# francescofugazzi/3dgsconverter

Measured on AMD Instinct MI355X. Metric: Msplats/sec SOR k=16, higher is better.
Workload: dtype f32 select / f64 finalize

## Files before the change

3dgsconverter_amd/_lib.py:

```python
from __future__ import annotations

import contextlib
import ctypes as C
import functools
import os
import re
import threading
import time

import numpy as np

_HERE = os.path.dirname(os.path.abspath(__file__))
LIB_PATH = os.environ.get("GSX_LIB_PATH") or os.path.join(_HERE, "libgsx_hip.so")

KNN_AUTO, KNN_BRUTE, KNN_GRID, KNN_TREE = 0, 1, 2, 3
PROBE_ROOT_DIST2, PROBE_ROOT_DSQRT = 0, 1
PROBE_MEAN_NET, PROBE_MEAN_LIST, PROBE_MEAN_LE128, PROBE_MEAN_NP = 0, 1, 2, 3
T_SOR_KNN, T_SOR_BIN, T_SOR_FALLBACK, T_SOR_STATS, T_DENSITY, T_KMEANS_ASSIGN, T_KMEANS_UPDATE, T_QUANTIZE = range(8)
T_SLAB_PREP, T_SLAB_ROWS, T_SLAB_MEANS, T_SLAB_COLL = range(8, 12)


class GsxError(RuntimeError):
    """Raised for every failure of the HIP path (missing library, no GPU, HIP error)."""

# ... 223 lines not shown
    "gsx_dev_download_staged": (_I, [_P, _P, _P, C.c_size_t]),
    "gsx_host_gather_f32": (_I, [_P, _I64, _I64, C.POINTER(_I64), _I, _P]),
    "gsx_host_gather_columns_f32": (_I, [_P, _I64, _I64, C.POINTER(_I64), _I, _P]),
    "gsx_host_compact_rows": (_I, [_P, _I64, _I64, _P, _P, _I64, C.POINTER(_I64)]),
    "gsx_host_take_rows": (_I, [_P, _I64, _I64, _P, _I64, _P]),
    "gsx_host_zero_columns": (_I, [_P, _I64, _I64, C.POINTER(_I64), _I]),
    "gsx_host_append_columns": (_I, [_P, _I64, _I64, _P, _I64, _P, _I64]),
    "gsx_host_take_rows_append": (_I, [_P, _I64, _I64, _P, _I64, _P, _I64, _P, _I64]),
    "gsx_host_take_rows_shape": (_I, [_P, _I64, _I64, _P, _I64, _P, _I64, C.POINTER(_I64), _I, _P, _I64]),
    "gsx_rgb_from_sh": (_I, [_P, _I64, _P, _P]),
    "gsx_rgb_from_sh_dev": (_I, [_P, _P, _I64, _P, _P]),
    "gsx_rgb_from_sh_list": (_I, [_P, _I64, _P, _P, _I64, C.POINTER(_I64)]),
    "gsx_rgb_from_sh_list_dev": (_I, [_P, _P, _I64, _P, _P, _I64, _P]),
    "gsx_compact_rows_dev": (_I, [_P, _P, _P, _P, _I64, _P, _P, C.POINTER(_I64)]),
    "gsx_mask_bbox_dev": (_I, [_P, _P, _I64, _P, _P]),
    "gsx_mask_ge_dev": (_I, [_P, _P, _P, _I64, _D, _P]),
    "gsx_sor_knn_dev": (_I, [_P, _P, _P, _P, _I64, _I64, _I64, _I64, _I, _I, _P, C.POINTER(SorInfo)]),
    "gsx_sor_knn_share_dev": (_I, [_P, _P, _P, _P, _I64, _I64, _I, _I, _I, _I, _P, C.POINTER(SorInfo)]),
    "gsx_sor_debug_brick_plan": (_I, [_P, _P, _P, _P, _I64]),
    "gsx_sor_debug_work_queue": (_I, [_P, _P, _P, _P]),
    "gsx_sor_debug_tree": (_I, [_P, _P, _P, _P, _I64, C.POINTER(_I64), C.POINTER(_I64)]),
    "gsx_sor_debug_wave_stamps": (_I, [_P, _I, _P, _I64, _P]),
    "gsx_sor_debug_points_per_cell": (_D, [_I, _I64, _I]),
    "gsx_sor_debug_group_bricks": (_I, [_P, _I64, _I, _I, _I, _P, C.POINTER(C.c_int32)]),
    "gsx_sor_debug_refine_sizing": (_I, [C.POINTER(RefineSizingIn), C.POINTER(RefineSizingOut)]),
    "gsx_knn_probe_root_dev": (_I, [_P, _P, _I64, _I, _P]),
    "gsx_knn_probe_mean_dev": (_I, [_P, _P, _I64, _I64, _I, _I, _I, _P]),
    "gsx_sor_stats_dev": (_I, [_P, _P, _I64, _D, _P]),
    "gsx_sor_mask_dev": (_I, [_P, _P, _I64, _P, _P]),
    "gsx_comm_unique_id": (_I, [_P]),
    "gsx_comm_init": (_I, [_P, _I, _I, _P]),
    "gsx_comm_destroy": (_I, [_P]),
    "gsx_comm_all_reduce": (_I, [_P, _P, _I64, _I]),
    "gsx_comm_all_gather": (_I, [_P, _P, _P, _I64]),
    "gsx_comm_all_to_all_v": (_I, [_P, _P, _P, _P, _P, _P, _P, _I]),
    "gsx_comm_all_to_all_segs": (_I, [_P, _P, _P, _I, _P, _P, _P, _P, _I]),
    "gsx_comm_abort": (_I, [_P]),
    "gsx_comm_transport": (_I, [_P]),
    "gsx_comm_rank": (_I, [_P, C.POINTER(_I), C.POINTER(_I)]),
    "gsx_comm_barrier": (_I, [_P]),
    "gsx_slab_plan": (_I, [_P, _I, _I, _I64, _I, _D, C.POINTER(SlabPlan)]),
    "gsx_sor_slab_step_dev": (_I, [_P, _P, _I64, _I, _D, _D, _P, C.POINTER(SlabStep)]),
    "gsx_slab_bbox_dev": (_I, [_P, _P, _P, _P, _I64, _I64, _P]),
    "gsx_slab_hist_dev": (_I, [_P, _P, _P, _P, _I64, _I64, _P, _P]),
    "gsx_slab_partition_dev": (_I, [_P, _P, _P, _P, _I64, _I64, _I, _I, C.c_float, C.c_float, _P, _I, _P, _P, _P, _P, _P]),
    "gsx_sor_knn_slab_dev": (_I, [_P, _P, _I64, _I64, _I, _P, _P]),
# ... 1985 lines not shown
        if sh_count:
            sh = np.stack([data["f_rest_%d" % j][rows] for j in range(sh_count)], axis=1)
            if level == 2:
                out["sh"] = np.clip((sh - -2.0) / (2.0 - -2.0) * 255, 0, 255).astype(np.uint8)
            else:
                out["sh"] = sh.astype(out.dtype["sh"].base)
    return out


def ksplat_centres_host(data: np.ndarray, bucket_size: int) -> np.ndarray:
    idx = np.arange(0, len(data), bucket_size)
    cols = []
    with np.errstate(all="ignore"):
        for a in "xyz":
            v = data[a]
            cols.append((np.minimum.reduceat(v, idx) + np.maximum.reduceat(v, idx)) / 2.0)
    return np.column_stack(cols).astype(np.float32)


def grid_points_per_cell(k: int, n: int, tuned: bool) -> float:
    return float(load().gsx_sor_debug_points_per_cell(int(k), int(n), int(bool(tuned))))


def grid_group_bricks(bricks, nbx: int, nby: int, nbz: int):
    b = np.array(bricks, dtype=np.uint32)
    sizes = np.zeros(8, np.uint32)
    ng = C.c_int32()
    check(load().gsx_sor_debug_group_bricks(b.ctypes.data, b.size, int(nbx), int(nby), int(nbz), sizes.ctypes.data, C.byref(ng)),
          "gsx_sor_debug_group_bricks")
    return b, [int(v) for v in sizes[:ng.value]]


def grid_refine_sizing(qb_lo, qb_hi, sub_queries: int, n_sub: int, pts_per_cell: float, parent_h: float, adaptive: int, hist,
                       bin_vol: float) -> RefineSizingOut:
    a = RefineSizingIn((C.c_float * 3)(*qb_lo), (C.c_float * 3)(*qb_hi), int(sub_queries), int(n_sub), float(pts_per_cell),
                       float(parent_h), int(adaptive), (C.c_uint32 * 32)(*[int(v) for v in hist]), float(bin_vol))
    out = RefineSizingOut()
    check(load().gsx_sor_debug_refine_sizing(C.byref(a), C.byref(out)), "gsx_sor_debug_refine_sizing")
    return out


def np_exp_host(x: np.ndarray) -> np.ndarray:
    x = np.ascontiguousarray(x, dtype=np.float32)
    out = np.empty_like(x)
    check(load().gsx_np_expf_host(x.ctypes.data, out.ctypes.data, x.size), "gsx_np_expf_host")
    return out
# ... 1659 lines not shown
```

3dgsconverter_amd/csrc/api.hip:

```cpp
#include <algorithm>
#include <mutex>

#include "grid_policy.h"
#include "gsx_common.h"
#include "gsx_internal.h"
#include "sor_grid_params.h"

namespace gsx {

static thread_local std::string g_err;

void set_error(const char *fmt, ...)
{
    char buf[1024];
    va_list ap;
    va_start(ap, fmt);
    vsnprintf(buf, sizeof(buf), fmt, ap);
    va_end(ap);
    g_err = buf;
}

int DevBuf::reserve(size_t bytes)
{
    if (bytes <= cap) return 0;
// ... 191 lines not shown
        s.used = 0;
        s.launches = 0;
        s.total_ms = 0.0;
    }
    return 0;
}

int gsx_ctx_get_timing(gsx_ctx *c, int slot, uint64_t *launches, double *total_ms)
{
    if (!c || slot < 0 || slot >= GSX_T_SLOTS) GSX_FAIL("gsx_ctx_get_timing: bad arguments");
    GSX_HIP(hipStreamSynchronize(c->stream));
    GSX_CHECK(timing_resolve(c, slot));
    if (launches) *launches = c->slots[slot].launches;
    if (total_ms) *total_ms = c->slots[slot].total_ms;
    return 0;
}

int gsx_ctx_set_param(gsx_ctx *c, const char *name, double value)
{
    if (!c || !name) GSX_FAIL("gsx_ctx_set_param: bad arguments");
    if (!strcmp(name, "grid_points_per_cell")) {
        if (value != 0.0 && !(value >= 1.0 && value <= 512.0)) GSX_FAIL("grid_points_per_cell must be 0 (auto) or in [1,512]");
        c->grid_points_per_cell = value;
    } else if (!strcmp(name, "brute_below")) {
        c->brute_below = (int64_t)value;
    } else if (!strcmp(name, "debug_skip")) {
#ifdef GSX_ABLATE
        c->debug_skip = (int)value;
#else
        if (value != 0.0) GSX_FAIL("debug_skip needs a profiling build of the library (-DGSX_ABLATE); this one computes exact results only");
#endif
    } else if (!strcmp(name, "kmeans_mfma")) {
        c->kmeans_mfma = value != 0.0;
    } else if (!strcmp(name, "km_exact_blocks")) {
        c->km_exact_blocks = value < 1 ? 1 : (value > 32 ? 32 : (int)value);
    } else if (!strcmp(name, "km_seg_rows")) {
        c->km_seg_rows = value >= 64 ? 64 : (value >= 32 ? 32 : 16);
    } else if (!strcmp(name, "km_group_mb")) {
        c->km_group_mb = value < 0 ? 0 : (int)value;
    } else if (!strcmp(name, "kmeans_cs")) {
        c->kmeans_cs = value != 0.0;
    } else if (!strcmp(name, "km_small_wgs")) {
        c->km_small_wgs = (int)value;
    } else if (!strcmp(name, "kmeans_cs_small")) {
        c->kmeans_cs_small = value != 0.0;
    } else if (!strcmp(name, "ring_fast")) {
// ... 157 lines not shown
#ifdef GSX_WAVE_STAMPS
    gsx::KnnWs &w = c->ws[0];
    if (!w.wavestamps.p) GSX_FAIL("gsx_sor_debug_wave_stamps: no grid KNN call has run on this context");
    GSX_HIP(hipSetDevice(c->device));
    GSX_HIP(hipStreamSynchronize(c->stream));
    const int64_t slots = c->ws_cap;
    const int64_t m = std::min<int64_t>(slots, cap);
    if (m > 0)
        GSX_HIP(hipMemcpy(out, (const uint64_t *)w.wavestamps.p + (size_t)kernel * slots * gsx::WS_WORDS,
                          sizeof(uint64_t) * gsx::WS_WORDS * (size_t)m, hipMemcpyDeviceToHost));
    *count = slots;
    return 0;
#else
    (void)cap;
    GSX_FAIL("gsx_sor_debug_wave_stamps needs a diagnostic build of the library (-DGSX_WAVE_STAMPS)");
#endif
}

double gsx_sor_debug_points_per_cell(int k, int64_t n, int tuned)
{
    return tuned ? gsx::grid_pts_per_cell(k, n) : gsx::grid_pts_per_cell_base(k, n);
}

int gsx_sor_debug_group_bricks(uint32_t *bricks, int64_t count, int nbx, int nby, int nbz, uint32_t *group_sizes, int32_t *n_groups)
{
    if (!bricks || !group_sizes || !n_groups || count < 0 || count > UINT32_MAX || nbx < 1 || nby < 1 || nbz < 1)
        GSX_FAIL("gsx_sor_debug_group_bricks: bad arguments");
    for (int64_t i = 0; i < count; ++i)
        if ((uint64_t)bricks[i] >= (uint64_t)nbx * nby * nbz) GSX_FAIL("gsx_sor_debug_group_bricks: brick %u outside the grid", bricks[i]);
    const std::vector<unsigned> sizes = gsx::group_deferred_bricks(bricks, (unsigned)count, nbx, nby, nbz);
    for (int g = 0; g < gsx::GRID_MAX_GROUPS; ++g) group_sizes[g] = g < (int)sizes.size() ? sizes[g] : 0u;
    *n_groups = (int32_t)sizes.size();
    return 0;
}

int gsx_sor_debug_refine_sizing(const gsx_refine_sizing_in *in, gsx_refine_sizing_out *out)
{
    if (!in || !out) GSX_FAIL("gsx_sor_debug_refine_sizing: null argument");
    const gsx::RefineClip r = gsx::refine_clip(in->qb_lo, in->qb_hi, in->sub_queries, in->pts_per_cell, in->parent_h, in->adaptive);
    *out = gsx_refine_sizing_out{r.nd3, r.probe_g, r.h_est, r.M, r.cert, {r.lo[0], r.lo[1], r.lo[2]}, {r.hi[0], r.hi[1], r.hi[2]}, r.r_cert,
                                 r.probe_g ? gsx::refine_probe_edge(in->hist, in->bin_vol, in->qb_lo, in->qb_hi, r.r_cert, in->n_sub,
                                                                    r.h_est, in->pts_per_cell)
                                           : 0.0};
    return 0;
}

// ... 504 lines not shown
```

3dgsconverter_amd/csrc/grid_policy.h:

```cpp
#pragma once

#include <algorithm>
#include <cmath>
#include <cstdint>
#include <unordered_map>
#include <vector>

namespace gsx {

constexpr int MAX_BUCKETS = 4096;
constexpr int MAX_BUCKET_CELLS = 4096;
constexpr int64_t GRID_MAX_CELLS = (int64_t)MAX_BUCKETS * MAX_BUCKET_CELLS - 64;

inline double grid_fill(int64_t n) { return n >= 4000000 ? 54.0 : 58.0; }

inline double grid_pts_per_cell_base(int k, int64_t n)
{
    double m = std::max(2.0, 0.47 * (double)(k + 1));
    const double fill = grid_fill(n);
    for (int cells = 8; cells >= 1; cells /= 2)
        if (m * cells > fill && m * cells <= 66.0) m = fill / cells;
    return m;
}

inline double grid_pts_per_cell(int k, int64_t n)
{
    double m = grid_pts_per_cell_base(k, n);
    const double fill = grid_fill(n);
    if (k >= 17 && k <= 20) m = std::min(m, fill / 8.0 + 0.375 * (double)std::max(0, k - 18));
    if (k >= 26 && k <= 31) m = std::min(m, 12.0 * fill / 54.0);
    if (k >= 35 && k <= 43) m = std::min(m, (k <= 38 ? 13.5 : 14.5) * fill / 54.0);
    if (k >= 44 && k <= 62) m = std::min(m, k <= 49 ? 16.0 : (k <= 58 ? 22.0 : 24.0));
    return m;
}

inline int64_t grid_cell_cap(int64_t n_ref) { return std::max<int64_t>(n_ref / 2, 64) + 64; }
inline int64_t grid_refine_cell_cap(int64_t n_ref) { return std::min<int64_t>(std::max<int64_t>(4 * n_ref, 64), GRID_MAX_CELLS) + 64; }

struct HistVerdict {
    unsigned fullest = 0, nonzero = 0;
    bool to_tree = false;
    bool no_deferral = false;
};
inline HistVerdict grid_hist_verdict(const unsigned *starts , int64_t n_ref, int nshares)
{
    HistVerdict v;
    for (int b = 0; b < MAX_BUCKETS; ++b) {
        const unsigned c = starts[b + 1] >= starts[b] ? starts[b + 1] - starts[b] : 0u;
        v.fullest = std::max(v.fullest, c);
        v.nonzero += c > 0;
    }
    v.to_tree = v.nonzero > 0 && (double)v.fullest > 3.0 * (double)n_ref / (double)v.nonzero;
    v.no_deferral = v.nonzero > 0 && (double)v.fullest <= 1.5 * (double)n_ref / (double)v.nonzero && nshares == 1;
    return v;
}

struct PlanCall {
    bool enabled;
    int level;
    bool whole_cloud;
// ... 120 lines not shown
```

3dgsconverter_amd/csrc/gsx_common.h:

```cpp
#pragma once

#include <hip/hip_runtime.h>

#include <cstdarg>
#include <cstdint>
#include <cstdio>
#include <cstring>
#include <string>
#include <vector>

#include "../../include/gsx_hip.h"
#include "dev_carve.h"

namespace gsx {

constexpr int WAVE = 64;

void set_error(const char *fmt, ...);

#define GSX_HIP(call)                                                                         \
    do {                                                                                      \
        hipError_t e__ = (call);                                                              \
        if (e__ != hipSuccess) {                                                              \
            gsx::set_error("%s failed: %s (%s:%d)", #call, hipGetErrorString(e__), __FILE__,  \
// ... 105 lines not shown
    PinnedBuf host;
};

struct TimingSlot {
    std::vector<hipEvent_t> ev;
    size_t used = 0;
    uint64_t launches = 0;
    double total_ms = 0.0;
};

}

struct gsx_ctx {
    int device = 0;
    hipStream_t stream = nullptr;
    hipStream_t owned_stream = nullptr;
    bool timing = false;
    unsigned timing_mask = 0xffffffffu;
    gsx::TimingSlot slots[GSX_T_SLOTS];
    int num_cu = 256;
    void *comm = nullptr;

    double grid_points_per_cell = 0.0;
    int64_t brute_below = 2048;
    int debug_skip = 0;
    int adaptive = 0;
    int defer_words = 64;
    int last_knn_algo = 0;
    int tree = 1;
    int kmeans_mfma = 1;
    int tree_leaf_cap = 0;
    int tree_cand_limit = 0;
    double tree_near_cell = 0.5;
    int tree_last_leaf_cap = 0;
    double tree_scale = 0.0;
    int km_exact_blocks = 4;
    int km_seg_rows = 32;
    int km_group_mb = 0;
    int km_small_wgs = 0;
    int kmeans_cs_small = 1;
    int kmeans_cs = 1;
    int ring_fast = 1;
    int phase2_net = 1;
    int brick_plan = 1;
    int ws_cap = 0;
    int wq_grid[4] = {0, 0, 0, 0};
// ... 30 lines not shown
```

3dgsconverter_amd/csrc/sor_grid.hip:

```cpp
#include <algorithm>
#include <chrono>
#include <cmath>
#include <cstdlib>
#include <type_traits>
#include <unordered_map>
#include <vector>

#include "grid_policy.h"
#include "gsx_common.h"
#include "gsx_internal.h"
#include "knn_common.h"
#include "knn_mfma.h"
#include "sor_grid_params.h"

namespace gsx {


constexpr int MAX_DIM = 1024;
#ifndef GSX_BUCKET_POINTS
#define GSX_BUCKET_POINTS 4096
#endif
constexpr int BUCKET_POINTS = GSX_BUCKET_POINTS;
#ifndef GSX_BIN_TILE
#define GSX_BIN_TILE 8192
#endif
constexpr int BIN_TILE = GSX_BIN_TILE;
constexpr int BRICK_THREADS = 256;
constexpr int HEAVY_RING_CANDIDATES = 1 << 16;
constexpr int HEAVY_CHUNK = 32768;
#ifndef GSX_WCAP_BIG
#define GSX_WCAP_BIG 32
#endif
#ifndef GSX_WCAP_MID
#define GSX_WCAP_MID 24
#endif
constexpr int WCAP = 24;

struct GridParamArgs {
    int n;
    double pts_per_cell;
    int cell_cap, debug_skip, share, nshares, defer_words;
    float parent_h;
    GridParams *gp;
    unsigned *devflags;
    double h_hint;
    int cert_axis;
    float cert_lo, cert_hi;
    unsigned *cert_count;
    int plan_req = 0, plan_cap = 0;
#ifdef GSX_WAVE_STAMPS
    unsigned long long *stamps = nullptr;
    int stamps_cap = 0;
#endif
};
__device__ void grid_params_body(const float *part, int nparts, const GridParamArgs &a);

__global__ __launch_bounds__(256) void bbox_partial_kernel(const float *__restrict__ x, const float *__restrict__ y,
                                                           const float *__restrict__ z, int64_t stride, int n,
                                                           float *__restrict__ part, GridParamArgs gpa)
{
    __shared__ float red[7][4];
    float mn[3] = {__builtin_inff(), __builtin_inff(), __builtin_inff()};
    float mx[3] = {-__builtin_inff(), -__builtin_inff(), -__builtin_inff()};
    float bad = 0.0f;
    const int step = gridDim.x * blockDim.x;
    for (int64_t i0 = blockIdx.x * blockDim.x + threadIdx.x; i0 < n; i0 += 4 * (int64_t)step) {
        float v[4][3];
#pragma unroll
        for (int u = 0; u < 4; ++u) {
            const int64_t i = (int64_t)(i0 + u * step < n ? i0 + u * step : i0) * stride;
            v[u][0] = x[i];
            v[u][1] = y[i];
            v[u][2] = z[i];
        }
#pragma unroll
        for (int u = 0; u < 4; ++u)
#pragma unroll
            for (int a = 0; a < 3; ++a) {
                mn[a] = fminf(mn[a], v[u][a]);
                mx[a] = fmaxf(mx[a], v[u][a]);
                bad = (fabsf(v[u][a]) < __builtin_inff()) ? bad : 1.0f;
            }
    }
#pragma unroll
    for (int a = 0; a < 3; ++a)
#pragma unroll
        for (int off = 32; off > 0; off >>= 1) {
            mn[a] = fminf(mn[a], __shfl_xor(mn[a], off));
            mx[a] = fmaxf(mx[a], __shfl_xor(mx[a], off));
// ... 65 lines not shown
        emax = e[a] > emax ? e[a] : emax;
    }
    double h;
    if (nd == 0 || !(emax < 1e300)) {
        h = 1.0;
    } else {
        double per = vol * pts_per_cell / (double)(n > 0 ? n : 1);
        h = nd == 3 ? cbrt(per) : (nd == 2 ? sqrt(per) : per);
        if (a.h_hint > 0.0 && a.h_hint < h) h = a.h_hint;
        double hmin = emax / (double)(MAX_DIM - 1);
        if (!(h > hmin)) h = hmin;
    }
    int nx, ny, nz;
    int bg = 1, bny = 1, bnz = 1;
    long long padded = 0;
    float inv_h;
    for (int it = 0; it < 256; ++it) {
        inv_h = (float)(1.0 / h);
        nx = (int)((v[3] - v[0]) * inv_h) + 1;
        ny = (int)((v[4] - v[1]) * inv_h) + 1;
        nz = (int)((v[5] - v[2]) * inv_h) + 1;
        bool ok = nx <= MAX_DIM && ny <= MAX_DIM && nz <= MAX_DIM && nx > 0 && ny > 0 && nz > 0;
        if (ok) {
            double per_row = (double)nx * pts_per_cell;
            bg = (int)(sqrt((double)BUCKET_POINTS / (per_row > 1.0 ? per_row : 1.0)) + 0.5);
            if (bg < 1) bg = 1;
            if (bg > (ny > nz ? ny : nz)) bg = ny > nz ? ny : nz;
            while (bg > 1 && (long long)bg * bg * nx > MAX_BUCKET_CELLS) --bg;
            for (;;) {
                bny = (ny + bg - 1) / bg;
                bnz = (nz + bg - 1) / bg;
                if ((long long)bny * bnz <= MAX_BUCKETS) break;
                ++bg;
            }
            padded = (long long)bny * bnz * bg * bg * nx;
            ok = (long long)bg * bg * nx <= MAX_BUCKET_CELLS && padded <= (long long)cell_cap;
        }
        if (ok) break;
        h *= 1.1;
    }
    bool bad = v[6] > 0.0f;
    for (int a = 0; a < 6; ++a) bad |= !(fabsf(v[a]) < 3.0e38f);
    if (bad || !(nx > 0 && ny > 0 && nz > 0) || padded <= 0 || padded > (long long)cell_cap ||
        (long long)bg * bg * nx > MAX_BUCKET_CELLS) {
        bad = true;
        nx = ny = nz = 1;
        bg = bny = bnz = 1;
        inv_h = 0.0f;
    }
    gp->ox = v[0]; gp->oy = v[1]; gp->oz = v[2];
    gp->inv_h = inv_h;
    gp->h = (float)h;
    gp->nx = nx; gp->ny = ny; gp->nz = nz;
    gp->bk_g = bg; gp->bk_ny = bny; gp->bk_nz = bnz;
    gp->bk_count = bny * bnz;
    gp->bk_cells = bg * bg * nx;
    gp->ncells = gp->bk_count * gp->bk_cells;
    int bdx = 2, bdy = 2, bdz = 2;
    if (pts_per_cell * 8.0 > 66.0) bdz = 1;
// ... 370 lines not shown
        if (j < hi - lo) {
            const float4 r = stage[j];
            out[tab[bucket_of(g, cell_coord(r.y, g.oy, g.inv_h, g.ny), cell_coord(r.z, g.oz, g.inv_h, g.nz))] + j] = r;
        }
    }
}

#ifndef GSX_SORT_THREADS
#define GSX_SORT_THREADS 512
#endif
#ifndef GSX_SORT_PPT
#define GSX_SORT_PPT 16
#endif
constexpr int SORT_THREADS = GSX_SORT_THREADS;
constexpr int SORT_PPT = GSX_SORT_PPT;
constexpr unsigned SORT_CAP = SORT_THREADS * SORT_PPT;

__device__ __forceinline__ int quarter_coord(float v, float o, float inv_h, int dim)
{
    int c = (int)((v - o) * (4.0f * inv_h));
    return min(max(c, 0), 4 * dim - 1);
}

template <bool FINE>
__global__ __launch_bounds__(SORT_THREADS) void bucket_sort_kernel(const GridParams *__restrict__ gp,
                                                          const unsigned *__restrict__ bk_start,
                                                          const float4 *__restrict__ in, float4 *__restrict__ out,
                                                          unsigned *__restrict__ cell_start, unsigned big_limit,
                                                          unsigned *__restrict__ fine_start)
{
    constexpr int SUB = FINE ? 4 : 1;
    __shared__ unsigned cnt[SUB * MAX_BUCKET_CELLS];
    __shared__ unsigned wsum[SORT_THREADS / 64];
    const GridParams g = *gp;
    const int b = blockIdx.x;
    if (g.bad_input || b >= g.bk_count) return;
    const int ncell = g.bk_cells;
    const int cells = SUB * ncell;
    const unsigned s0 = bk_start[b], s1 = bk_start[b + 1];
    if (b == g.bk_count - 1 && threadIdx.x == 0) {
        cell_start[(size_t)g.bk_count * ncell] = s1;
        if (FINE) fine_start[(size_t)g.bk_count * cells] = s1;
    }
    if (s1 - s0 > big_limit) return;
    const int by = b % g.bk_ny, bz = b / g.bk_ny;
    for (int i = threadIdx.x; i < cells; i += SORT_THREADS) cnt[i] = 0;
    __syncthreads();
    auto local_cell = [&](const float4 p) {
        const int cx = FINE ? quarter_coord(p.x, g.ox, g.inv_h, g.nx) : cell_coord(p.x, g.ox, g.inv_h, g.nx);
        const int cy = cell_coord(p.y, g.oy, g.inv_h, g.ny);
        const int cz = cell_coord(p.z, g.oz, g.inv_h, g.nz);
        return ((cz - bz * g.bk_g) * g.bk_g + (cy - by * g.bk_g)) * (SUB * g.nx) + cx;
    };
    const bool fits = s1 - s0 <= SORT_CAP;
    float4 p[SORT_PPT];
    int cell[SORT_PPT];
    unsigned rk[SORT_PPT];
    if (fits) {
#pragma unroll
        for (int u = 0; u < SORT_PPT; ++u) p[u] = in[min(s0 + u * SORT_THREADS + threadIdx.x, s1 - 1)];
#pragma unroll
        for (int u = 0; u < SORT_PPT; ++u) {
            cell[u] = local_cell(p[u]);
            rk[u] = s0 + u * SORT_THREADS + threadIdx.x < s1 ? atomicAdd(&cnt[cell[u]], 1u) : 0u;
        }
    } else {
        for (unsigned i = s0 + threadIdx.x; i < s1; i += SORT_THREADS) atomicAdd(&cnt[local_cell(in[i])], 1u);
    }
    __syncthreads();
    const int seg = (cells + SORT_THREADS - 1) / SORT_THREADS;
    const int c0 = min(cells, (int)threadIdx.x * seg), c1 = min(cells, c0 + seg);
    unsigned sum = 0;
    for (int c = c0; c < c1; ++c) sum += cnt[c];
    unsigned inc = sum;
#pragma unroll
    for (int off = 1; off < 64; off <<= 1) {
        unsigned o = __shfl_up(inc, off);
        if ((int)(threadIdx.x & 63) >= off) inc += o;
    }
    const int wv = threadIdx.x >> 6;
    if ((threadIdx.x & 63) == 63) wsum[wv] = inc;
    __syncthreads();
    unsigned run = inc - sum;
    for (int i = 0; i < wv; ++i) run += wsum[i];
    __syncthreads();
    for (int c = c0; c < c1; ++c) {
        const unsigned v = cnt[c];
        cnt[c] = run;
        run += v;
    }
    __syncthreads();
    unsigned *cs = cell_start + (size_t)b * ncell;
    for (int i = threadIdx.x; i < ncell; i += SORT_THREADS) cs[i] = s0 + cnt[SUB * i];
    if (FINE) {
        unsigned *fs = fine_start + (size_t)b * cells;
        for (int i = threadIdx.x; i < cells; i += SORT_THREADS) fs[i] = s0 + cnt[i];
    }
    if (fits) {
#pragma unroll
        for (int u = 0; u < SORT_PPT; ++u)
            if (s0 + u * SORT_THREADS + threadIdx.x < s1) out[s0 + cnt[cell[u]] + rk[u]] = p[u];
    } else {
        __syncthreads();
        for (unsigned i = s0 + threadIdx.x; i < s1; i += SORT_THREADS) {
            const float4 q = in[i];
            out[s0 + atomicAdd(&cnt[local_cell(q)], 1u)] = q;
        }
    }
}

constexpr unsigned BIG_BUCKET = 32768;
constexpr int BIG_CHUNK = 8192;

__device__ __forceinline__ int bucket_containing(const unsigned *bk_start, int nb, unsigned pos)
{
    int lo = 0, hi = nb;
    while (hi - lo > 1) {
        const int mid = (lo + hi) >> 1;
        if (bk_start[mid] <= pos) lo = mid; else hi = mid;
    }
    return lo;
}

template <bool SCATTER>
__global__ __launch_bounds__(256) void big_bucket_kernel(const GridParams *__restrict__ gp, const unsigned *__restrict__ bk_start,
                                                         int n, const float4 *__restrict__ in, float4 *__restrict__ out,
                                                         unsigned *cell_start ,
                                                         unsigned *cursor )
{
    __shared__ unsigned cnt[MAX_BUCKET_CELLS];
    __shared__ unsigned base[SCATTER ? MAX_BUCKET_CELLS : 1];
// ... 1907 lines not shown
    if (L.adaptive) {
        GSX_CHECK(w.deferred.reserve(sizeof(unsigned) * (size_t)(cap + 64)));
        GSX_CHECK(w.heavylist.reserve(sizeof(unsigned) * (size_t)std::max<int64_t>(q_count, 1)));
    }
    if (!L.all) {
        GSX_CHECK(w.qsorted.reserve(sizeof(float4) * (size_t)q_count));
        GSX_CHECK(w.qcellstart.reserve(sizeof(unsigned) * (size_t)(cap + 1)));
    }
    L.gp = w.gridparams.as<GridParams>();
    L.refs = w.packed.as<float4>();
    L.rstart = w.cellstart.as<unsigned>();
    L.mfma_ok = ctx->filter_mfma != 0 && n_ref < (int64_t(1) << 28);
    L.plan = grid_plan_eligible({ctx->brick_plan != 0, L.level, L.all, L.slab, L.sk != nullptr, L.nshares, L.k, L.mfma_ok,
                                 ctx->phase2_net != 0, L.pts_per_cell, L.h_hint, L.kth_out != nullptr});
    L.plan_cap = n_ref / 16 + 4096;
    if (L.plan) {
        GSX_CHECK(w.finestart.reserve(sizeof(unsigned) * (size_t)(4 * cap + 4)));
        GSX_CHECK(w.bricklist.reserve(sizeof(uint2) * (size_t)L.plan_cap));
        GSX_CHECK(w.bundleoff.reserve(sizeof(unsigned) * 2 * (size_t)(MAX_DIM / 2) * (MAX_DIM / 2)));
    }
    return 0;
}

static int level_grid_params(GridLevel &L)
{
    gsx_ctx *ctx = L.ctx;
    KnnWs &w = L.w;
    const SlabKnn *sk = L.sk;
    GSX_CHECK(timing_begin(ctx, GSX_T_SOR_BIN));
    GridParamArgs gpa{(int)L.n_ref, L.pts_per_cell, (int)L.cap, ctx->debug_skip, L.share, L.nshares, L.adaptive ? ctx->defer_words : 0,
                      L.parent_h, L.gp, ctx->devflags.as<unsigned>(), L.h_hint, sk ? sk->cert_axis : -1, sk ? sk->cert_lo : 0.0f,
                      sk ? sk->cert_hi : 0.0f, sk ? sk->cert_count : nullptr, L.plan ? 1 : 0, (int)L.plan_cap};
#ifdef GSX_WAVE_STAMPS
    if (L.level == 0) {
        const int ws_cap = ctx->num_cu * 8 * (BRICK_THREADS / 64);
        const size_t ws_bytes = sizeof(unsigned long long) * 2 * (size_t)ws_cap * WS_WORDS;
        GSX_CHECK(w.wavestamps.reserve(ws_bytes));
        GSX_HIP(hipMemsetAsync(w.wavestamps.p, 0, ws_bytes, ctx->stream));
        gpa.stamps = w.wavestamps.as<unsigned long long>();
        gpa.stamps_cap = ws_cap;
        ctx->ws_cap = ws_cap;
    }
#endif
    L.adaptive_at_bbox = L.adaptive;
    if (sk && sk->box.b7)
        hipLaunchKernelGGL(grid_params_known_box_kernel, dim3(1), dim3(64), 0, ctx->stream, sk->box, w.bboxpart.as<float>(), gpa);
    else
        hipLaunchKernelGGL(bbox_partial_kernel, dim3(L.bbox_blocks), dim3(256), 0, ctx->stream, L.x, L.y, L.z, L.stride, (int)L.n_ref,
                           w.bboxpart.as<float>(), gpa);
    GSX_HIP(hipGetLastError());
    if (L.adaptive) GSX_CHECK(w.qcellstart.reserve(sizeof(unsigned) * (size_t)(L.cap + 1)));
    return 0;
}

static int level_histogram(GridLevel &L, bool *done)
{
    gsx_ctx *ctx = L.ctx;
    KnnWs &w = L.w;
    L.tree_ok = (L.adaptive || (L.slab && ctx->adaptive)) && ctx->tree && L.level == 0 && L.k + 1 <= 65 && L.n_ref > L.k;
    if (!L.tree_ok) return 0;
    GSX_CHECK(bin_hist(ctx, w, L.x, L.y, L.z, L.stride, 0, L.n_ref, L.gp));
    static thread_local std::vector<unsigned> starts(MAX_BUCKETS + 1);
    GSX_HIP(hipMemcpyAsync(starts.data(), w.bk_start, sizeof(unsigned) * (MAX_BUCKETS + 1), hipMemcpyDeviceToHost, ctx->stream));
    GSX_HIP(hipStreamSynchronize(ctx->stream));
    const HistVerdict v = grid_hist_verdict(starts.data(), L.n_ref, L.nshares);
    L.hist_done = true;
    if (v.to_tree) {
        GSX_CHECK(timing_end(ctx, GSX_T_SOR_BIN));
        if (L.trace)
            fprintf(stderr, "[gsx] level 0: fullest bucket %u of %lld points in %u buckets -> tree path\n", v.fullest, (long long)L.n_ref, v.nonzero);
        const int rc = launch_knn_tree(ctx, L.x, L.y, L.z, L.stride, L.n_ref, L.q_begin, L.q_count, L.k, L.mean_out, L.kth_out, L.info,
                                       L.slab ? L.ref_only_from : INT32_MAX, L.share, L.nshares, true);
// ... 284 lines not shown
```

include/gsx_hip.h:

```cpp
#ifndef GSX_HIP_H
#define GSX_HIP_H

#include <stddef.h>
#include <stdint.h>

#ifdef __cplusplus
extern "C" {
#endif

typedef struct gsx_ctx gsx_ctx;

enum {
    GSX_KNN_AUTO = 0,
    GSX_KNN_BRUTE = 1,
    GSX_KNN_GRID = 2,
    GSX_KNN_TREE = 3
};

enum {
    GSX_T_SOR_KNN = 0,
    GSX_T_SOR_BIN = 1,
    GSX_T_SOR_FALLBACK = 2,
    GSX_T_SOR_STATS = 3,
    GSX_T_DENSITY = 4,
// ... 69 lines not shown
                            void *out, int64_t out_row_bytes);
int gsx_host_take_rows_append(const void *rows, int64_t row_bytes, int64_t n, const uint32_t *idx, int64_t n_idx,
                              const uint8_t *extra, int64_t extra_bytes, void *out, int64_t out_row_bytes);
int gsx_host_take_rows_shape(const void *rows, int64_t row_bytes, int64_t n, const uint32_t *idx, int64_t n_idx,
                             const uint8_t *extra, int64_t extra_bytes, const int64_t *zero_offsets, int nzero, void *out,
                             int64_t out_row_bytes);

int gsx_mask_bbox_dev(gsx_ctx *ctx, const float *rows_dev, int64_t n, const double *bounds6, uint8_t *mask_dev);
int gsx_mask_ge_dev(gsx_ctx *ctx, const float *vals_dev, const uint32_t *orig_dev, int64_t n, double threshold,
                    uint8_t *mask_dev);

int gsx_sor_knn_dev(gsx_ctx *ctx, const float *x, const float *y, const float *z, int64_t stride,
                    int64_t n_ref, int64_t q_begin, int64_t q_count, int k, int algo,
                    float *mean_out_dev, gsx_sor_info *info );
int gsx_sor_knn_share_dev(gsx_ctx *ctx, const float *x, const float *y, const float *z, int64_t stride,
                          int64_t n, int k, int algo, int share, int nshares, float *mean_out_dev,
                          gsx_sor_info *info );
int gsx_sor_debug_brick_plan(gsx_ctx *ctx, int32_t *grid, float *origin, uint32_t *list, int64_t cap);
int gsx_sor_debug_work_queue(gsx_ctx *ctx, uint32_t *ctr, int64_t *items, int32_t *blocks);
int gsx_sor_debug_tree(gsx_ctx *ctx, uint32_t *counters, uint64_t *keys, uint32_t *leafstart, int64_t cap, int64_t *n_out,
                       int64_t *leaves_out);
int gsx_sor_debug_wave_stamps(gsx_ctx *ctx, int kernel, uint64_t *out, int64_t cap, int64_t *count);
double gsx_sor_debug_points_per_cell(int k, int64_t n, int tuned);
int gsx_sor_debug_group_bricks(uint32_t *bricks, int64_t count, int nbx, int nby, int nbz, uint32_t *group_sizes, int32_t *n_groups);
typedef struct gsx_refine_sizing_in {
    float    qb_lo[3], qb_hi[3];
    uint32_t sub_queries, n_sub;
    double   pts_per_cell;
    float    parent_h;
    int32_t  adaptive;
    uint32_t hist[32];
    double   bin_vol;
} gsx_refine_sizing_in;
typedef struct gsx_refine_sizing_out {
    int32_t nd3, probe_g;
    double  h_est, margin, cert;
    float   clip_lo[3], clip_hi[3], r_cert;
    double  h_hint;
} gsx_refine_sizing_out;
int gsx_sor_debug_refine_sizing(const gsx_refine_sizing_in *in, gsx_refine_sizing_out *out);
enum { GSX_PROBE_ROOT_DIST2 = 0, GSX_PROBE_ROOT_DSQRT = 1 };
int gsx_knn_probe_root_dev(gsx_ctx *ctx, const double *in_dev, int64_t n, int mode, double *out_dev);
enum { GSX_PROBE_MEAN_NET = 0, GSX_PROBE_MEAN_LIST = 1, GSX_PROBE_MEAN_LE128 = 2, GSX_PROBE_MEAN_NP = 3 };
int gsx_knn_probe_mean_dev(gsx_ctx *ctx, const double *d2_dev, int64_t m, int64_t stride, int k, int form, int cap,
                           float *out_dev);
int gsx_sor_stats_dev(gsx_ctx *ctx, const float *mean_dists_dev, int64_t n, double threshold_factor,
// ... 496 lines not shown
```

Before: 6229.

## Vectorize bbox reduction for packed rows and specialize bucket sort per fill

When x, y and z are interleaved with stride 3 and 16-byte aligned, the bbox partial kernel now reads them as float4 rows with unrolled wave-wide loads and un-rotates the per-lane axes afterwards. The bucket sort kernel now dispatches to template instantiations sized to the actual number of points per thread, so under-filled buckets skip wasted register loads. Bucket edge sizing is factored into a shared host/device helper with a runtime bucket_points parameter and a debug entry point. The specialization adds several kernel instantiations, which grows code size and may raise register pressure.

```diff
diff --git a/3dgsconverter_amd/_lib.py b/3dgsconverter_amd/_lib.py
--- a/3dgsconverter_amd/_lib.py
+++ b/3dgsconverter_amd/_lib.py
@@ -269,6 +269,7 @@
     "gsx_sor_debug_tree": (_I, [_P, _P, _P, _P, _I64, C.POINTER(_I64), C.POINTER(_I64)]),
     "gsx_sor_debug_wave_stamps": (_I, [_P, _I, _P, _I64, _P]),
     "gsx_sor_debug_points_per_cell": (_D, [_I, _I64, _I]),
+    "gsx_sor_debug_bucket_edge": (_I, [_I, _I, _I, _D, _I, _I64, _P]),
     "gsx_sor_debug_group_bricks": (_I, [_P, _I64, _I, _I, _I, _P, C.POINTER(C.c_int32)]),
     "gsx_sor_debug_refine_sizing": (_I, [C.POINTER(RefineSizingIn), C.POINTER(RefineSizingOut)]),
     "gsx_knn_probe_root_dev": (_I, [_P, _P, _I64, _I, _P]),
@@ -2300,6 +2301,13 @@
     return float(load().gsx_sor_debug_points_per_cell(int(k), int(n), int(bool(tuned))))
 
 
+def grid_bucket_edge(nx: int, ny: int, nz: int, pts_per_cell: float, bucket_points: int = 0, cell_cap: int = 1 << 40):
+    out = np.zeros(5, np.int64)
+    check(load().gsx_sor_debug_bucket_edge(int(nx), int(ny), int(nz), float(pts_per_cell), int(bucket_points), int(cell_cap),
+                                           out.ctypes.data), "gsx_sor_debug_bucket_edge")
+    return int(out[0]), int(out[1]), int(out[2]), int(out[3]), bool(out[4])
+
+
 def grid_group_bricks(bricks, nbx: int, nby: int, nbz: int):
     b = np.array(bricks, dtype=np.uint32)
     sizes = np.zeros(8, np.uint32)
diff --git a/3dgsconverter_amd/csrc/api.hip b/3dgsconverter_amd/csrc/api.hip
--- a/3dgsconverter_amd/csrc/api.hip
+++ b/3dgsconverter_amd/csrc/api.hip
@@ -237,6 +237,9 @@
     if (!strcmp(name, "grid_points_per_cell")) {
         if (value != 0.0 && !(value >= 1.0 && value <= 512.0)) GSX_FAIL("grid_points_per_cell must be 0 (auto) or in [1,512]");
         c->grid_points_per_cell = value;
+    } else if (!strcmp(name, "bucket_points")) {
+        if (value != 0.0 && !(value >= 64.0 && value <= 1048576.0)) GSX_FAIL("bucket_points must be 0 (built in) or in [64,1048576]");
+        c->bucket_points = (int)value;
     } else if (!strcmp(name, "brute_below")) {
         c->brute_below = (int64_t)value;
     } else if (!strcmp(name, "debug_skip")) {
@@ -440,6 +443,14 @@
     return tuned ? gsx::grid_pts_per_cell(k, n) : gsx::grid_pts_per_cell_base(k, n);
 }
 
+int gsx_sor_debug_bucket_edge(int nx, int ny, int nz, double pts_per_cell, int bucket_points, int64_t cell_cap, int64_t out[5])
+{
+    if (!out || nx < 1 || ny < 1 || nz < 1 || bucket_points < 0) GSX_FAIL("gsx_sor_debug_bucket_edge: bad arguments");
+    const gsx::BucketEdge e = gsx::grid_bucket_edge(nx, ny, nz, pts_per_cell, bucket_points, (long long)cell_cap);
+    out[0] = e.bg; out[1] = e.bny; out[2] = e.bnz; out[3] = e.padded; out[4] = e.ok ? 1 : 0;
+    return 0;
+}
+
 int gsx_sor_debug_group_bricks(uint32_t *bricks, int64_t count, int nbx, int nby, int nbz, uint32_t *group_sizes, int32_t *n_groups)
 {
     if (!bricks || !group_sizes || !n_groups || count < 0 || count > UINT32_MAX || nbx < 1 || nby < 1 || nbz < 1)
diff --git a/3dgsconverter_amd/csrc/grid_policy.h b/3dgsconverter_amd/csrc/grid_policy.h
--- a/3dgsconverter_amd/csrc/grid_policy.h
+++ b/3dgsconverter_amd/csrc/grid_policy.h
@@ -5,6 +5,12 @@
 #include <cstdint>
 #include <unordered_map>
 #include <vector>
+
+#if defined(__HIPCC__)
+#define GSX_POLICY_HD __host__ __device__
+#else
+#define GSX_POLICY_HD
+#endif
 
 namespace gsx {
 
@@ -36,6 +42,34 @@
 
 inline int64_t grid_cell_cap(int64_t n_ref) { return std::max<int64_t>(n_ref / 2, 64) + 64; }
 inline int64_t grid_refine_cell_cap(int64_t n_ref) { return std::min<int64_t>(std::max<int64_t>(4 * n_ref, 64), GRID_MAX_CELLS) + 64; }
+
+#ifndef GSX_BUCKET_POINTS
+#define GSX_BUCKET_POINTS 4096
+#endif
+constexpr int BUCKET_POINTS = GSX_BUCKET_POINTS;
+struct BucketEdge {
+    int bg, bny, bnz;
+    long long padded;
+    bool ok;
+};
+GSX_POLICY_HD inline BucketEdge grid_bucket_edge(int nx, int ny, int nz, double pts_per_cell, int bucket_points, long long cell_cap)
+{
+    BucketEdge e;
+    const double per_row = (double)nx * pts_per_cell;
+    e.bg = (int)(sqrt((double)(bucket_points > 0 ? bucket_points : BUCKET_POINTS) / (per_row > 1.0 ? per_row : 1.0)) + 0.5);
+    if (e.bg < 1) e.bg = 1;
+    if (e.bg > (ny > nz ? ny : nz)) e.bg = ny > nz ? ny : nz;
+    while (e.bg > 1 && (long long)e.bg * e.bg * nx > MAX_BUCKET_CELLS) --e.bg;
+    for (;;) {
+        e.bny = (ny + e.bg - 1) / e.bg;
+        e.bnz = (nz + e.bg - 1) / e.bg;
+        if ((long long)e.bny * e.bnz <= MAX_BUCKETS) break;
+        ++e.bg;
+    }
+    e.padded = (long long)e.bny * e.bnz * e.bg * e.bg * nx;
+    e.ok = (long long)e.bg * e.bg * nx <= MAX_BUCKET_CELLS && e.padded <= cell_cap;
+    return e;
+}
 
 struct HistVerdict {
     unsigned fullest = 0, nonzero = 0;
diff --git a/3dgsconverter_amd/csrc/gsx_common.h b/3dgsconverter_amd/csrc/gsx_common.h
--- a/3dgsconverter_amd/csrc/gsx_common.h
+++ b/3dgsconverter_amd/csrc/gsx_common.h
@@ -151,6 +151,7 @@
     void *comm = nullptr;
 
     double grid_points_per_cell = 0.0;
+    int bucket_points = 0;
     int64_t brute_below = 2048;
     int debug_skip = 0;
     int adaptive = 0;
diff --git a/3dgsconverter_amd/csrc/sor_grid.hip b/3dgsconverter_amd/csrc/sor_grid.hip
--- a/3dgsconverter_amd/csrc/sor_grid.hip
+++ b/3dgsconverter_amd/csrc/sor_grid.hip
@@ -17,10 +17,6 @@
 
 
 constexpr int MAX_DIM = 1024;
-#ifndef GSX_BUCKET_POINTS
-#define GSX_BUCKET_POINTS 4096
-#endif
-constexpr int BUCKET_POINTS = GSX_BUCKET_POINTS;
 #ifndef GSX_BIN_TILE
 #define GSX_BIN_TILE 8192
 #endif
@@ -48,6 +44,7 @@
     float cert_lo, cert_hi;
     unsigned *cert_count;
     int plan_req = 0, plan_cap = 0;
+    int bucket_points = 0;
 #ifdef GSX_WAVE_STAMPS
     unsigned long long *stamps = nullptr;
     int stamps_cap = 0;
@@ -57,14 +54,51 @@
 
 __global__ __launch_bounds__(256) void bbox_partial_kernel(const float *__restrict__ x, const float *__restrict__ y,
                                                            const float *__restrict__ z, int64_t stride, int n,
-                                                           float *__restrict__ part, GridParamArgs gpa)
+                                                           float *__restrict__ part, GridParamArgs gpa, int rows)
 {
     __shared__ float red[7][4];
     float mn[3] = {__builtin_inff(), __builtin_inff(), __builtin_inff()};
     float mx[3] = {-__builtin_inff(), -__builtin_inff(), -__builtin_inff()};
     float bad = 0.0f;
     const int step = gridDim.x * blockDim.x;
-    for (int64_t i0 = blockIdx.x * blockDim.x + threadIdx.x; i0 < n; i0 += 4 * (int64_t)step) {
+    int64_t done = 0;
+    if (rows) {
+        const float4 *v4 = reinterpret_cast<const float4 *>(x);
+        const int lane = threadIdx.x & 63;
+        const int64_t rounds = n / 256, waves = (int64_t)gridDim.x * (blockDim.x >> 6);
+        float amn[3] = {__builtin_inff(), __builtin_inff(), __builtin_inff()};
+        float amx[3] = {-__builtin_inff(), -__builtin_inff(), -__builtin_inff()};
+        constexpr int RU = 3;
+        for (int64_t r0 = (int64_t)blockIdx.x * (blockDim.x >> 6) + (threadIdx.x >> 6); r0 < rounds; r0 += RU * waves) {
+            float4 t[RU][3];
+#pragma unroll
+            for (int q = 0; q < RU; ++q) {
+                const int64_t r = r0 + q * waves < rounds ? r0 + q * waves : r0;
+#pragma unroll
+                for (int j = 0; j < 3; ++j) t[q][j] = v4[r * 192 + 64 * j + lane];
+            }
+#pragma unroll
+            for (int q = 0; q < RU; ++q)
+#pragma unroll
+                for (int j = 0; j < 3; ++j) {
+                    const float e4[4] = {t[q][j].x, t[q][j].y, t[q][j].z, t[q][j].w};
+#pragma unroll
+                    for (int e = 0; e < 4; ++e) {
+                        amn[(j + e) % 3] = fminf(amn[(j + e) % 3], e4[e]);
+                        amx[(j + e) % 3] = fmaxf(amx[(j + e) % 3], e4[e]);
+                        bad = (fabsf(e4[e]) < __builtin_inff()) ? bad : 1.0f;
+                    }
+                }
+        }
+        const int m = lane % 3;
+#pragma unroll
+        for (int c = 0; c < 3; ++c) {
+            mn[c] = m == 0 ? amn[c] : (m == 1 ? amn[(c + 2) % 3] : amn[(c + 1) % 3]);
+            mx[c] = m == 0 ? amx[c] : (m == 1 ? amx[(c + 2) % 3] : amx[(c + 1) % 3]);
+        }
+        done = rounds * 256;
+    }
+    for (int64_t i0 = done + blockIdx.x * blockDim.x + threadIdx.x; i0 < n; i0 += 4 * (int64_t)step) {
         float v[4][3];
 #pragma unroll
         for (int u = 0; u < 4; ++u) {
@@ -176,19 +210,10 @@
         nz = (int)((v[5] - v[2]) * inv_h) + 1;
         bool ok = nx <= MAX_DIM && ny <= MAX_DIM && nz <= MAX_DIM && nx > 0 && ny > 0 && nz > 0;
         if (ok) {
-            double per_row = (double)nx * pts_per_cell;
-            bg = (int)(sqrt((double)BUCKET_POINTS / (per_row > 1.0 ? per_row : 1.0)) + 0.5);
-            if (bg < 1) bg = 1;
-            if (bg > (ny > nz ? ny : nz)) bg = ny > nz ? ny : nz;
-            while (bg > 1 && (long long)bg * bg * nx > MAX_BUCKET_CELLS) --bg;
-            for (;;) {
-                bny = (ny + bg - 1) / bg;
-                bnz = (nz + bg - 1) / bg;
-                if ((long long)bny * bnz <= MAX_BUCKETS) break;
-                ++bg;
-            }
-            padded = (long long)bny * bnz * bg * bg * nx;
-            ok = (long long)bg * bg * nx <= MAX_BUCKET_CELLS && padded <= (long long)cell_cap;
+            const BucketEdge e = grid_bucket_edge(nx, ny, nz, pts_per_cell, a.bucket_points, (long long)cell_cap);
+            bg = e.bg; bny = e.bny; bnz = e.bnz;
+            padded = e.padded;
+            ok = e.ok;
         }
         if (ok) break;
         h *= 1.1;
@@ -605,27 +630,15 @@
     return min(max(c, 0), 4 * dim - 1);
 }
 
-template <bool FINE>
-__global__ __launch_bounds__(SORT_THREADS) void bucket_sort_kernel(const GridParams *__restrict__ gp,
-                                                          const unsigned *__restrict__ bk_start,
-                                                          const float4 *__restrict__ in, float4 *__restrict__ out,
-                                                          unsigned *__restrict__ cell_start, unsigned big_limit,
-                                                          unsigned *__restrict__ fine_start)
+template <bool FINE, int NU>
+__device__ __forceinline__ void bucket_sort_body(const GridParams &g, int b, unsigned s0, unsigned s1, const float4 *__restrict__ in,
+                                                 float4 *__restrict__ out, unsigned *__restrict__ cell_start,
+                                                 unsigned *__restrict__ fine_start, unsigned *cnt, unsigned *wsum)
 {
     constexpr int SUB = FINE ? 4 : 1;
-    __shared__ unsigned cnt[SUB * MAX_BUCKET_CELLS];
-    __shared__ unsigned wsum[SORT_THREADS / 64];
-    const GridParams g = *gp;
-    const int b = blockIdx.x;
-    if (g.bad_input || b >= g.bk_count) return;
+    constexpr int NS = NU > 0 ? NU : 1;
     const int ncell = g.bk_cells;
     const int cells = SUB * ncell;
-    const unsigned s0 = bk_start[b], s1 = bk_start[b + 1];
-    if (b == g.bk_count - 1 && threadIdx.x == 0) {
-        cell_start[(size_t)g.bk_count * ncell] = s1;
-        if (FINE) fine_start[(size_t)g.bk_count * cells] = s1;
-    }
-    if (s1 - s0 > big_limit) return;
     const int by = b % g.bk_ny, bz = b / g.bk_ny;
     for (int i = threadIdx.x; i < cells; i += SORT_THREADS) cnt[i] = 0;
     __syncthreads();
@@ -635,15 +648,14 @@
         const int cz = cell_coord(p.z, g.oz, g.inv_h, g.nz);
         return ((cz - bz * g.bk_g) * g.bk_g + (cy - by * g.bk_g)) * (SUB * g.nx) + cx;
     };
-    const bool fits = s1 - s0 <= SORT_CAP;
-    float4 p[SORT_PPT];
-    int cell[SORT_PPT];
-    unsigned rk[SORT_PPT];
-    if (fits) {
-#pragma unroll
-        for (int u = 0; u < SORT_PPT; ++u) p[u] = in[min(s0 + u * SORT_THREADS + threadIdx.x, s1 - 1)];
-#pragma unroll
-        for (int u = 0; u < SORT_PPT; ++u) {
+    float4 p[NS];
+    int cell[NS];
+    unsigned rk[NS];
+    if (NU > 0) {
+#pragma unroll
+        for (int u = 0; u < NU; ++u) p[u] = in[min(s0 + u * SORT_THREADS + threadIdx.x, s1 - 1)];
+#pragma unroll
+        for (int u = 0; u < NU; ++u) {
             cell[u] = local_cell(p[u]);
             rk[u] = s0 + u * SORT_THREADS + threadIdx.x < s1 ? atomicAdd(&cnt[cell[u]], 1u) : 0u;
         }
@@ -679,9 +691,9 @@
         unsigned *fs = fine_start + (size_t)b * cells;
         for (int i = threadIdx.x; i < cells; i += SORT_THREADS) fs[i] = s0 + cnt[i];
     }
-    if (fits) {
-#pragma unroll
-        for (int u = 0; u < SORT_PPT; ++u)
+    if (NU > 0) {
+#pragma unroll
+        for (int u = 0; u < NU; ++u)
             if (s0 + u * SORT_THREADS + threadIdx.x < s1) out[s0 + cnt[cell[u]] + rk[u]] = p[u];
     } else {
         __syncthreads();
@@ -690,6 +702,39 @@
             out[s0 + atomicAdd(&cnt[local_cell(q)], 1u)] = q;
         }
     }
+}
+
+template <bool FINE, int NU = 1, typename... A>
+__device__ __forceinline__ void bucket_sort_dispatch(int used, A &&...a)
+{
+    if constexpr (NU > SORT_PPT) {
+        bucket_sort_body<FINE, 0>(a...);
+    } else {
+        if (used == NU) bucket_sort_body<FINE, NU>(a...);
+        else bucket_sort_dispatch<FINE, NU + 1>(used, a...);
+    }
+}
+
+template <bool FINE>
+__global__ __launch_bounds__(SORT_THREADS) void bucket_sort_kernel(const GridParams *__restrict__ gp,
+                                                          const unsigned *__restrict__ bk_start,
+                                                          const float4 *__restrict__ in, float4 *__restrict__ out,
+                                                          unsigned *__restrict__ cell_start, unsigned big_limit,
+                                                          unsigned *__restrict__ fine_start)
+{
+    constexpr int SUB = FINE ? 4 : 1;
+    __shared__ unsigned cnt[SUB * MAX_BUCKET_CELLS];
+    __shared__ unsigned wsum[SORT_THREADS / 64];
+    const GridParams g = *gp;
+    const int b = blockIdx.x;
+    if (g.bad_input || b >= g.bk_count) return;
+    const unsigned s0 = bk_start[b], s1 = bk_start[b + 1];
+    if (b == g.bk_count - 1 && threadIdx.x == 0) {
+        cell_start[(size_t)g.bk_count * g.bk_cells] = s1;
+        if (FINE) fine_start[(size_t)g.bk_count * SUB * g.bk_cells] = s1;
+    }
+    if (s1 - s0 > big_limit) return;
+    bucket_sort_dispatch<FINE>((int)((s1 - s0 + SORT_THREADS - 1) / SORT_THREADS), g, b, s0, s1, in, out, cell_start, fine_start, cnt, wsum);
 }
 
 constexpr unsigned BIG_BUCKET = 32768;
@@ -2643,6 +2688,11 @@
     return 0;
 }
 
+static bool bbox_rows_layout(const float *x, const float *y, const float *z, int64_t stride)
+{
+    return stride == 3 && y == x + 1 && z == x + 2 && (reinterpret_cast<uintptr_t>(x) & 15u) == 0;
+}
+
 static int level_grid_params(GridLevel &L)
 {
     gsx_ctx *ctx = L.ctx;
@@ -2651,7 +2701,7 @@
     GSX_CHECK(timing_begin(ctx, GSX_T_SOR_BIN));
     GridParamArgs gpa{(int)L.n_ref, L.pts_per_cell, (int)L.cap, ctx->debug_skip, L.share, L.nshares, L.adaptive ? ctx->defer_words : 0,
                       L.parent_h, L.gp, ctx->devflags.as<unsigned>(), L.h_hint, sk ? sk->cert_axis : -1, sk ? sk->cert_lo : 0.0f,
-                      sk ? sk->cert_hi : 0.0f, sk ? sk->cert_count : nullptr, L.plan ? 1 : 0, (int)L.plan_cap};
+                      sk ? sk->cert_hi : 0.0f, sk ? sk->cert_count : nullptr, L.plan ? 1 : 0, (int)L.plan_cap, ctx->bucket_points};
 #ifdef GSX_WAVE_STAMPS
     if (L.level == 0) {
         const int ws_cap = ctx->num_cu * 8 * (BRICK_THREADS / 64);
@@ -2668,7 +2718,7 @@
         hipLaunchKernelGGL(grid_params_known_box_kernel, dim3(1), dim3(64), 0, ctx->stream, sk->box, w.bboxpart.as<float>(), gpa);
     else
         hipLaunchKernelGGL(bbox_partial_kernel, dim3(L.bbox_blocks), dim3(256), 0, ctx->stream, L.x, L.y, L.z, L.stride, (int)L.n_ref,
-                           w.bboxpart.as<float>(), gpa);
+                           w.bboxpart.as<float>(), gpa, bbox_rows_layout(L.x, L.y, L.z, L.stride) ? 1 : 0);
     GSX_HIP(hipGetLastError());
     if (L.adaptive) GSX_CHECK(w.qcellstart.reserve(sizeof(unsigned) * (size_t)(L.cap + 1)));
     return 0;
diff --git a/include/gsx_hip.h b/include/gsx_hip.h
--- a/include/gsx_hip.h
+++ b/include/gsx_hip.h
@@ -115,6 +115,7 @@
                        int64_t *leaves_out);
 int gsx_sor_debug_wave_stamps(gsx_ctx *ctx, int kernel, uint64_t *out, int64_t cap, int64_t *count);
 double gsx_sor_debug_points_per_cell(int k, int64_t n, int tuned);
+int gsx_sor_debug_bucket_edge(int nx, int ny, int nz, double pts_per_cell, int bucket_points, int64_t cell_cap, int64_t out[5]);
 int gsx_sor_debug_group_bricks(uint32_t *bricks, int64_t count, int nbx, int nby, int nbz, uint32_t *group_sizes, int32_t *n_groups);
 typedef struct gsx_refine_sizing_in {
     float    qb_lo[3], qb_hi[3];
```

After: 6244, median of 6. Within noise of the previous version (+0.2%).
